# plsakr/rna-sequence-diff-patch

Measured on AMD Instinct MI355X. Metric: DP cells/sec (whole node) + edit-script bit-exact rate, 4k×4k RNA pairs, higher is better.
Workload: dtype u32

## Files before the change

### include/sed.h

```cpp
#ifndef SED_H
#define SED_H
#include <stdint.h>

#ifdef __cplusplus
extern "C" {
#endif

enum {
    SED_OK = 0,
    SED_E_ARG = -1,
    SED_E_DEVICE = -2,
    SED_E_OOM = -3,
    SED_E_RANGE = -4,
    SED_E_ALPHABET = -5,
    SED_E_STATE = -6
};

#define SED_WANT_SCRIPT 1u
#define SED_PIPELINE 2u
#define SED_NO_LEN 4u

#define SED_OPT_MODE 1
#define SED_OPT_ROWS_PER_LANE 2
#define SED_OPT_SPLIT 3
// ... 48 lines not shown
                            const uint8_t *codes_b, const int64_t *off_b, const int32_t *len_b,
                            int32_t npairs, uint32_t flags);
void sed_batch_destroy(sed_batch *b);
int sed_batch_mode(const sed_batch *b);
int sed_batch_rows_per_lane(const sed_batch *b);
int sed_batch_lane_pairs(const sed_batch *b);
int sed_batch_chains(const sed_batch *b);
int sed_batch_packed_pairs(const sed_batch *b);
int sed_batch_bitpar_pairs(const sed_batch *b);
int sed_batch_scaled_pairs(const sed_batch *b);
int sed_batch_segment_pairs(const sed_batch *b);
int sed_batch_split_tasks(const sed_batch *b);
int sed_dot_factor(const double *sub, double ins, double del, int maxmin, int ladder_maxsum, uint32_t *out);
#define SED_PLAN_ENV_TBPAR 101
#define SED_PLAN_ENV_BAND 102
#define SED_PLAN_ENV_ALT_DP 103
#define SED_PLAN_ENV_CK_HALVES 104
int sed_plan_routes(int K, const double *sub, const uint8_t *sub_int, double ins, int ins_is_int, double del,
                    int del_is_int, const int32_t *options, int noptions,
                    const uint8_t *codes_a, const int64_t *off_a, const int32_t *len_a,
                    const uint8_t *codes_b, const int64_t *off_b, const int32_t *len_b,
                    int32_t npairs, uint32_t flags, double *out, int nout);
int sed_batch_dot_keys(const sed_batch *b);
int sed_band_refine_row(int32_t n, int32_t m, int32_t rows_per_lane, double ins, double del, int32_t stripe,
                        double ub_prev, double suf, const int32_t *drow, int32_t clo_prev, int32_t chi_prev,
                        int32_t *out);
double sed_batch_band_chunks_run(sed_batch *b, double *total);
int sed_band_bounds(int32_t n, int32_t m, double ins, double del, double ub, int32_t *out);
int sed_band_chunk_range(int32_t n, int32_t m, int32_t rows_per_lane, int32_t elo, int32_t ehi, int32_t stripe,
                         int32_t *out);
double sed_band_cells(const double *sub, double ins, double del, const uint8_t *codes_a, int32_t n,
                      const uint8_t *codes_b, int32_t m, int32_t rows_per_lane);
double sed_batch_band_cells(const sed_batch *b);
int sed_batch_set_cutoff(sed_batch *b, double max_dist);
int sed_batch_cutoff_hits(sed_batch *b, int32_t *within);
int sed_batch_traceback_mode(const sed_batch *b);
int sed_batch_chain_stats(sed_batch *b, int32_t *fetched, int32_t *max_per_wave);
int sed_batch_run(sed_batch *b);
int sed_batch_sync(sed_batch *b);
int sed_batch_dp_launches(const sed_batch *b);
int sed_batch_last_times(const sed_batch *b, float *dp_ms, float *traceback_ms);
int sed_batch_times(sed_batch *b, float *dp_ms, float *traceback_ms, int max_runs);
int sed_batch_spans(sed_batch *b, float *out, int max_runs);
int sed_batch_reset_times(sed_batch *b);
int sed_batch_set_timing(sed_batch *b, int every);
int sed_batch_results(sed_batch *b, double *out_dist, uint8_t *out_is_int, int32_t *out_len,
                      uint32_t *out_ops, const int64_t *ops_off);
int sed_batch_device_results(const sed_batch *b, uint64_t *d_dist, uint64_t *d_is_int,
                             uint64_t *d_len, uint64_t *d_ops, uint64_t *ops_words);
int sed_batch_export(sed_batch *b, uint64_t d_dist, uint64_t d_len, uint64_t d_ops);
int sed_batch_work(const sed_batch *b, double *cells, double *algo_bytes);

int sed_fit_search(sed_ctx *ctx,
                   const uint8_t *codes_p, const int64_t *off_p, const int32_t *len_p,
                   const uint8_t *codes_t, const int64_t *off_t, const int32_t *len_t,
                   int32_t npairs, double *out_dist, int32_t *out_start, int32_t *out_end);
int sed_fit_plan(int K, const double *sub, const uint8_t *sub_int, double ins, int ins_is_int,
                 double del, int del_is_int, const int32_t *options, int noptions,
                 const int32_t *len_p, const int32_t *len_t, int32_t npairs, double *out, int nout);
int sed_fit_lanes(int K, const double *sub, const uint8_t *sub_int, double ins, int ins_is_int,
                  double del, int del_is_int, const int32_t *options, int noptions,
                  const int32_t *len_p, const int32_t *len_t, int32_t npairs,
                  int32_t *out_lanes, int64_t max_lanes, uint32_t *out_params);
int sed_fit_last_time(const sed_ctx *ctx, float *kernel_ms);

typedef struct sed_fit_index sed_fit_index;
// ... 34 lines not shown
```

### rna-sequence-diff-patch_amd/csrc/sed_internal.h

```cpp
#pragma once
#include <hip/hip_runtime.h>
#include <stdint.h>

#define SED_MAX_K 32

struct sed_pair_desc {
    uint64_t a_off;
    uint64_t b_off;
    uint64_t tb_off;
    uint64_t bnd_off;
    uint64_t ops_off;
    int32_t n, m;
    int32_t lane;
    int32_t map_off;
    int32_t pad[2];
};

struct sed_result {
    double dist;
    int32_t len;
    uint8_t is_int;
    uint8_t err;
    uint16_t seq;
};
// ... 53 lines not shown
    double ins, del;
    int32_t ins_int, del_int;
    int32_t K;
    uint32_t epoch;
};

struct sed_full_out {
    double *D;
    uint8_t *M;
    int32_t n, m;
};

#define SED_LAUNCH(kernel, grid, block, shmem, L, ...) \
    hipExtLaunchKernelGGL(kernel, grid, block, shmem, (L).stream, (L).ev0, (L).ev1, 0, __VA_ARGS__)

struct sed_launch {
    const sed_pair_desc *pd;
    int npairs;
    const void *seqa, *seqb;
    uint32_t *tb;
    uint32_t *ops;
    uint32_t *bnd;
    sed_result *res;
    int R;
    hipStream_t stream;
    bool tb_ladder;
    bool tb_wide;
    bool ck;
    struct sed_band *band;
    const struct sed_band_params *bandp;
    int2 *bwin;
    uint32_t *bsuf;
    int bstripes;
    hipEvent_t ev0, ev1;
    const int2 *tasks;
    int ntasks;
    const int32_t *chain_pairs, *chain_off;
    int nchains;
    uint32_t *chain_counter;
    uint32_t chain_base;
    int chain_list;
};

hipError_t sed_launch_i32(const sed_launch &L, const sed_i32_params &prm, bool len);
hipError_t sed_launch_i32_chain(const sed_launch &L, const sed_i32_params &prm, bool len);
hipError_t sed_launch_f64(const sed_launch &L, const double *gtab, const sed_f64_params &prm, bool typed);
hipError_t sed_launch_f64_seg(const sed_launch &L, const double *gtab, const sed_f64_params &prm, bool typed,
                              const int32_t *idx, int nidx);
hipError_t sed_launch_traceback_seg(const sed_launch &L, uint32_t *ops, const int32_t *idx, int nidx);
hipError_t sed_launch_f64_full(const sed_launch &L, const double *gtab, const sed_f64_params &prm, bool typed,
                               const sed_full_out &fo);
#define SED_LANE_MAXM 32
#define SED_LANE_MAXN 512
hipError_t sed_launch_lane_i32(const sed_launch &L, const int32_t *idx, int nidx, const sed_i32_params &prm, bool len);
hipError_t sed_launch_i32x2(const sed_launch &L, const int32_t *list, int nwaves, const sed_i32_params &prm);
hipError_t sed_launch_lane_i32x2(const sed_launch &L, const int32_t *idx, int nlanes, const sed_i32_params &prm);
hipError_t sed_launch_lane_bitpar(const sed_launch &L, const int32_t *idx, int nidx);
hipError_t sed_launch_lane_f64(const sed_launch &L, const int32_t *idx, int nidx, const double *gtab, double ins,
                               double del, int K, uint32_t umask);
struct sed_scaled_params {
    uint32_t row[8][2];
    uint32_t ins, del;
    double inv_scale;
    uint32_t umask, umap;
};
hipError_t sed_launch_lane_scaled(const sed_launch &L, const int32_t *idx, int nidx, const sed_scaled_params &sp);
// ... 137 lines not shown
    if (any) {
        const uint32_t us = (uint32_t)s;
        const int32_t elo = lo >= 0 ? (int32_t)(((uint32_t)lo + us - 1u) / us) : -(int32_t)((uint32_t)(-lo) / us);
        const int32_t ehi = hi >= 0 ? (int32_t)((uint32_t)hi / us) : -(int32_t)(((uint32_t)(-hi) + us - 1u) / us);
        w.elo = elo > w.elo ? elo : w.elo;
        w.ehi = ehi < w.ehi ? ehi : w.ehi;
    }
    sed_band_chunks(n, m, ROWS, nchunks, w, k, clo, chi);
    *clo = *clo > clo_prev ? *clo : clo_prev;
    *chi = *chi > chi_prev ? *chi : chi_prev;
    return any;
}
struct sed_stripe_wins {
    int2 *win;
    const uint32_t *suf;
    int stride;
};
__host__ __device__ inline double sed_band_pair_cells(int n, int m, int R, sed_band w) {
    const int ROWS = 64 * R, nstripes = sed_stripe_geom(n, m, R, 64).nstripes, nchunks = sed_stripe_geom(n, m, R, 64).nchunks;
    double cells = 0;
    for (int k = 0; k < nstripes; ++k) {
        int clo, chi;
        sed_band_chunks(n, m, ROWS, nchunks, w, k, &clo, &chi);
        const int rows = (k + 1) * ROWS < n ? ROWS : n - k * ROWS;
        const int jend = (chi >= nchunks - 1 || 64 * chi > m) ? m : 64 * chi;
        cells += (double)rows * (double)(jend - 64 * clo);
    }
    return cells;
}
struct sed_band_params {
    uint32_t cost[16];
    uint32_t ins, del;
};
hipError_t sed_launch_band(const sed_launch &L, const sed_band_params &bp);
hipError_t sed_launch_cut_band(const sed_launch &L, const int32_t *list, int nlist, uint32_t *diag,
                               const sed_band_params &bp, uint32_t tkey);
hipError_t sed_launch_i32_cut(const sed_launch &L, const int32_t *list, int nlist, const sed_i32_params &prm,
                              uint32_t tkey);
hipError_t sed_launch_cut_filter(const sed_launch &L, double cutoff, uint32_t *hits);
hipError_t sed_launch_traceback_ck(const sed_launch &L, uint32_t *ops, const sed_i32_params &prm);
hipError_t sed_launch_ck_codes(const sed_launch &L, int max_tiles, const sed_i32_params &prm);
hipError_t sed_launch_selftest(uint32_t *d_out, hipStream_t stream);
```

### rna-sequence-diff-patch_amd/csrc/sed_kernels.hip

```cpp
#include <hip/hip_ext.h>
#include <stdlib.h>
#include "sed_ck_tile.h"

template <int R> struct I32Waves { static constexpr int value = R >= 32 ? 4 : (R == 16 ? 5 : 7); };
#ifndef SED_SPLIT_BWORDS
#define SED_SPLIT_BWORDS 1024
#endif
#ifndef SED_CK_WAVES
#define SED_CK_WAVES 5
#endif
#ifndef SED_CK_GUNROLL
#define SED_CK_GUNROLL 2
#endif
#ifdef SED_I32_WAVES_PER_EU
#define SED_I32_WAVES(R) SED_I32_WAVES_PER_EU
#else
#define SED_I32_WAVES(R) I32Waves<R>::value
#endif

#define SED_SPLIT_RING 256
template <int G>
__device__ __forceinline__ void split_feed(const uint64_t *__restrict__ bin64, const int m, const int SG,
                                           const uint32_t epoch, uint32_t *ring, uint32_t *flag,
                                           const int lane) {
// ... 1280 lines not shown
    const int n = d.n, m = d.m;
    if (d.lane || n == 0 || m == 0) {
        if (lane == 0) band[pair] = sed_band{SED_BAND_OPEN_LO, SED_BAND_OPEN_HI};
        return;
    }
    const uint32_t gap = m > n ? (uint32_t)(m - n) * bp.ins : (uint32_t)(n - m) * bp.del;
    uint32_t sum = 0;
    if (suf) {
        const int len = min(n, m), words = (len + 15) >> 4, wps = ROWS >> 4;
        const uint32_t *pa = seqa + d.a_off, *pb = seqb + d.b_off;
        uint32_t *out = suf + (size_t)pair * stride;
        for (int k = (n + ROWS - 1) / ROWS - 1; k >= 0; --k) {
            uint32_t part = 0;
            for (int w = k * wps + lane; w < min(words, (k + 1) * wps); w += 64) {
                uint32_t x = pa[w], y = pb[w];
                const int cnt = min(16, len - 16 * w);
                for (int u = 0; u < cnt; ++u) {
                    part += tab[((x & 3u) << 2) | (y & 3u)];
                    x >>= 2;
                    y >>= 2;
                }
            }
#pragma unroll
            for (int o = 32; o > 0; o >>= 1) part += __shfl_xor(part, o);
            sum += part;
            if (lane == 0) out[k] = k * ROWS <= len ? sum + gap : SED_REFINE_NO_SUF;
        }
    } else {
        sum = diag_cost_sum(tab, seqa + d.a_off, seqb + d.b_off, min(n, m), lane);
    }
    if (lane == 0) band[pair] = sed_band_window(n, m, bp.ins, bp.del, (uint64_t)sum + gap);
}

__global__ __launch_bounds__(256) void sed_cut_band_kernel(const sed_pair_desc *__restrict__ pd,
                                                           const int32_t *__restrict__ list, int nlist,
                                                           const uint32_t *__restrict__ seqa,
                                                           const uint32_t *__restrict__ seqb, sed_band *__restrict__ band,
                                                           uint32_t *__restrict__ diag, sed_band_params bp, uint32_t tkey) {
    __shared__ uint32_t tab[16];
    diag_cost_table(tab, bp);
    const int lane = threadIdx.x & 63;
    const int w = blockIdx.x * 4 + (threadIdx.x >> 6);
    if (w >= nlist) return;
    const int pair = list[w];
    const sed_pair_desc d = pd[pair];
    const int n = d.n, m = d.m;
    if (n == 0 || m == 0) {
        if (lane == 0) {
            band[pair] = sed_band{SED_BAND_OPEN_LO, SED_BAND_OPEN_HI};
            if (diag) diag[pair] = 0xFFFFFFFFu;
        }
        return;
    }
    const uint32_t sum = diag_cost_sum(tab, seqa + d.a_off, seqb + d.b_off, min(n, m), lane);
    if (lane == 0) {
        const uint64_t gap = m > n ? (uint64_t)(m - n) * bp.ins : (uint64_t)(n - m) * bp.del;
        const uint64_t ub = (uint64_t)sum + gap;
        if (diag) diag[pair] = (uint32_t)(ub < 0xFFFFFFFFull ? ub : 0xFFFFFFFFull);
        band[pair] = gap > (uint64_t)tkey ? sed_band{1, 0}
                                          : sed_band_window(n, m, bp.ins, bp.del, ub < (uint64_t)tkey ? ub : (uint64_t)tkey);
    }
}

__global__ __launch_bounds__(256) void sed_cut_filter_kernel(sed_result *__restrict__ res, int npairs, double cutoff,
                                                             uint32_t *__restrict__ hits) {
    const int p = blockIdx.x * 256 + threadIdx.x;
// ... 18 lines not shown
    if (nlist <= 0) return hipSuccess;
    hipExtLaunchKernelGGL(sed_cut_band_kernel, dim3((nlist + 3) / 4), dim3(256), 0, L.stream, L.ev0, nullptr, 0, L.pd, list,
                          nlist, (const uint32_t *)L.seqa, (const uint32_t *)L.seqb, L.band, diag, bp, tkey);
    return hipGetLastError();
}
hipError_t sed_launch_i32_cut(const sed_launch &L, const int32_t *list, int nlist, const sed_i32_params &prm,
                              uint32_t tkey) {
    if (nlist <= 0 || !L.band || !L.bandp) return hipErrorInvalidValue;
    const hipError_t e = sed_launch_cut_band(L, list, nlist, nullptr, *L.bandp, tkey);
    if (e != hipSuccess) return e;
    sed_launch Lf = L;
    Lf.ev0 = nullptr;
    const dim3 grid((nlist + 3) / 4), block(256);
    const int2 *lp = reinterpret_cast<const int2 *>(list);
    const uint32_t *a = (const uint32_t *)L.seqa, *b = (const uint32_t *)L.seqb;
    switch (L.R) {
#define CASE(RR)                                                                                                        \
    case RR:                                                                                                            \
        SED_LAUNCH((sed_wf_i32_kernel<RR, false, false, false, false, false, true>), grid, block, 0, Lf, L.pd, nlist, lp, a, \
                   b, (uint32_t *)nullptr, L.bnd, L.res, prm, (const sed_band *)L.band, sed_stripe_wins{});             \
        break;
        CASE(4) CASE(8) CASE(16)
#undef CASE
    default: return hipErrorInvalidValue;
    }
    return hipGetLastError();
}
hipError_t sed_launch_cut_filter(const sed_launch &L, double cutoff, uint32_t *hits) {
    if (L.npairs <= 0) return hipSuccess;
    SED_LAUNCH(sed_cut_filter_kernel, dim3((L.npairs + 255) / 256), dim3(256), 0, L, L.res, L.npairs, cutoff, hits);
    return hipGetLastError();
}
hipError_t sed_launch_band(const sed_launch &L, const sed_band_params &bp) {
    hipExtLaunchKernelGGL(sed_band_kernel, dim3((L.npairs + 3) / 4), dim3(256), 0, L.stream, L.ev0, nullptr, 0, L.pd,
                          L.npairs, (const uint32_t *)L.seqa, (const uint32_t *)L.seqb, L.band, bp, L.bsuf, L.bstripes,
                          64 * L.R);
    return hipGetLastError();
}
template <int R, bool TB, bool LEN = true, bool CK = false, bool DOT = false>
static hipError_t launch_i32_R(const sed_launch &L, const sed_i32_params &prm) {
    if (L.ntasks > 0) {
        if constexpr (CK && R != 4) {
            return hipErrorInvalidValue;
        } else {
            SED_LAUNCH((sed_wf_i32_kernel<R, TB, true, LEN, CK, DOT>), dim3(L.ntasks), dim3(128), 0, L, L.pd, L.npairs,
                       L.tasks, (const uint32_t *)L.seqa, (const uint32_t *)L.seqb, L.tb, L.bnd, L.res, prm,
                       (const sed_band *)nullptr, sed_stripe_wins{});
        }
    } else {
        const int grid = (L.npairs + 3) / 4;
        static const int occ_lds = [] { const char *e = getenv("SED_OCC_LDS"); return e ? atoi(e) : 0; }();
        sed_launch Lf = L;
        if (CK && L.band && L.bandp) {
            const hipError_t e = sed_launch_band(L, *L.bandp);
            if (e != hipSuccess) return e;
            Lf.ev0 = nullptr;
        }
        SED_LAUNCH((sed_wf_i32_kernel<R, TB, false, LEN, CK, DOT>), dim3(grid), dim3(256), occ_lds, Lf, L.pd, L.npairs,
                           L.tasks, (const uint32_t *)L.seqa, (const uint32_t *)L.seqb, L.tb, L.bnd, L.res,
                           prm, CK ? (const sed_band *)L.band : nullptr,
                           CK && L.band ? sed_stripe_wins{L.bwin, L.bsuf, L.bstripes} : sed_stripe_wins{});
    }
    return hipGetLastError();
}

template <int R, bool TB, bool LEN, bool CK = false, int LDOT = 0>
// ... 146 lines not shown
```

### rna-sequence-diff-patch_amd/csrc/sed_plan.cpp

```cpp
#include "sed_plan.h"

#include <algorithm>
#include <climits>
#include <cmath>
#include <cstdarg>
#include <cstdio>
#include <cstring>

int sed_plan_fail(std::string *err, int code, const char *fmt, ...) {
    char buf[512];
    va_list ap;
    va_start(ap, fmt);
    vsnprintf(buf, sizeof buf, fmt, ap);
    va_end(ap);
    if (err) *err = buf;
    return code;
}

namespace {

bool is_integral_small(double v, int lim) { return v == std::floor(v) && v >= 0 && v < lim; }

struct DotKeys {
    bool ok = false;
// ... 983 lines not shown
    for (const OptSpec &s : env_table)
        if (env_keys && s.key == key) {
            o.*s.field = value;
            return true;
        }
    return false;
}

bool sed_simple_typing(const sed_costs &c) {
    if (c.ins_int || c.del_int || !(c.ins > 0) || !(c.del > 0)) return false;
    for (int e = 0; e < c.K * c.K; ++e) {
        if (c.sub_int[e] ? c.sub[e] != 0 : !(c.sub[e] > 0)) return false;
    }
    return true;
}

sed_band_params sed_band_params_from(const sed_costs &c) {
    sed_band_params bp{};
    for (int a = 0; a < 4; ++a)
        for (int bb = 0; bb < 4; ++bb)
            bp.cost[a * 4 + bb] = (a < c.K && bb < c.K) ? (uint32_t)c.sub[a * c.K + bb] : 0u;
    bp.ins = (uint32_t)c.ins;
    bp.del = (uint32_t)c.del;
    return bp;
}

uint64_t sed_band_diag_bound(const sed_band_params &bp, const uint8_t *a, int n, const uint8_t *b, int m) {
    uint64_t ub = 0;
    const int len = std::min(n, m);
    for (int i = 0; i < len; ++i) ub += bp.cost[(a[i] & 3) * 4 + (b[i] & 3)];
    return ub + (m > n ? (uint64_t)(m - n) * bp.ins : (uint64_t)(n - m) * bp.del);
}

int sed_plan_batch(const sed_costs &c, const sed_opts &o, const uint8_t *codes_a, const int64_t *off_a,
                   const int32_t *len_a, const uint8_t *codes_b, const int64_t *off_b, const int32_t *len_b,
                   int32_t npairs, uint32_t flags, sed_plan *plan, std::string *err) {
    Planning P{c, o, codes_a, off_a, len_a, codes_b, off_b, len_b, npairs, flags, *plan, err};
    int rc = plan_validate(P);
    if (rc != SED_OK) return rc;
    plan->npairs = npairs;
    plan->flags = flags;
    P.want_tb = (flags & SED_WANT_SCRIPT) != 0;
    if ((rc = plan_mode(P)) != SED_OK) return rc;
    plan_traceback(P);
    plan_layout(P);
    const bool x2_ok = plan->mode == SED_MODE_I32 && x2_costs_ok(c);
    plan_lane_routes(P, x2_ok);
    plan_wave_x2(P, x2_ok);
    plan_chain(P);
    plan_band(P);
    plan_params(P);
    plan_buffers(P);
    return SED_OK;
}

void sed_pack_sequences(const sed_plan &plan, const uint8_t *codes_a, const int64_t *off_a, const int32_t *len_a,
                        const uint8_t *codes_b, const int64_t *off_b, const int32_t *len_b, std::vector<uint32_t> &ha,
                        std::vector<uint32_t> &hb) {
    ha.assign((plan.up_copy[SED_UP_SEQA] + 3) / 4, 0);
    hb.assign((plan.up_copy[SED_UP_SEQB] + 3) / 4, 0);
    for (int p = 0; p < plan.npairs; ++p) {
        const sed_pair_desc &d = plan.pd[p];
        if (plan.mode == SED_MODE_I32) {
            pack2(codes_a + off_a[p], len_a[p], ha.data() + d.a_off);
            pack2(codes_b + off_b[p], len_b[p], hb.data() + d.b_off);
        } else {
// ... 100 lines not shown
    const int R = rows_per_lane;
    if (!out || n < 1 || m < 1 || (R != 4 && R != 8 && R != 16) || stripe < 0 || stripe >= sed_stripe_geom(n, m, R, 64).nstripes)
        return SED_E_ARG;
    const int nchunks = sed_stripe_geom(n, m, R, 64).nchunks;
    int clo, chi;
    sed_band_chunks(n, m, 64 * R, nchunks, sed_band{elo, ehi}, stripe, &clo, &chi);
    out[0] = clo;
    out[1] = chi;
    out[2] = nchunks;
    return SED_OK;
}

double sed_band_cells(const double *sub, double ins, double del, const uint8_t *codes_a, int32_t n,
                      const uint8_t *codes_b, int32_t m, int32_t rows_per_lane) {
    const int R = rows_per_lane;
    if (!sub || !codes_a || !codes_b || n < 1 || m < 1 || (R != 4 && R != 8 && R != 16) || !(ins >= 0) || !(del >= 0) ||
        !(ins + del > 0) || ins >= 65536 || del >= 65536)
        return -1.0;
    for (int i = 0; i < 16; ++i)
        if (!(sub[i] >= 0) || sub[i] >= 65536) return -1.0;
    sed_costs c;
    c.K = 4;
    c.sub.assign(sub, sub + 16);
    c.ins = ins;
    c.del = del;
    const sed_band_params bp = sed_band_params_from(c);
    for (int i = 0; i < n; ++i)
        if (codes_a[i] > 3) return -1.0;
    for (int i = 0; i < m; ++i)
        if (codes_b[i] > 3) return -1.0;
    return sed_band_pair_cells(n, m, R, sed_band_window(n, m, bp.ins, bp.del, sed_band_diag_bound(bp, codes_a, n, codes_b, m)));
}

}
```

### rna-sequence-diff-patch_amd/csrc/sed_plan.h

```cpp
#pragma once
#include "../../include/sed.h"
#include "sed_internal.h"

#include <string>
#include <vector>

struct sed_costs {
    int K = 0;
    std::vector<double> sub;
    std::vector<uint8_t> sub_int;
    double ins = 1, del = 1;
    int ins_int = 0, del_int = 0;
};

struct sed_opts {
    int mode = 0, R = 0, split = 0, lane = 0, chain = 0, pack = 0, tb = 0;
    int chain_waves = 0;
    int bitpar = 0;
    int scaled = 0;
    int seg = 0;
    int splitck = 0;
    int zc = 0;
    int dot = 0;
    int debug_corrupt = 0;
    int band = 0;
    int cut = 0;
    int fit_chunk = 0;
    int env_tbpar = -1;
    int env_band = 1;
    int env_alt_dp = 1;
    int env_ck_halves = -1;
};
bool sed_opts_set(sed_opts &o, int key, int value, bool env_keys);

int sed_plan_fail(std::string *err, int code, const char *fmt, ...);

#define SED_SMALL_BATCH_BYTES (4u << 20)

enum { SED_UP_PD, SED_UP_SEQA, SED_UP_SEQB, SED_UP_TASKS, SED_UP_CHAIN, SED_UP_LANE, SED_UP_X2, SED_UP_SEG, SED_UP_COUNT };

struct sed_plan {
    int npairs = 0;
    uint32_t flags = 0;
    int mode = 0, R = 0;
    bool split = false;
    bool ck = false;
    bool split_ck = false;
    int ck_tiles = 0;
    bool tbpar = false;
    int tbpar_items = 0, tbpar_kmax = 0;
    bool band = false;
    bool band_refine = false;
    int band_stripes = 0;
    sed_band_params bandp{};
    double band_cells = 0;
    bool cut_costs_ok = false;
    sed_band_params cut_bp{};
    bool dot = false;
    bool lad = false;
    int nlane = 0, nwave = 0;
    int nlane_x2 = 0;
    bool lane_bitpar = false;
// ... 3 lines not shown
    sed_scaled_params sp{};
    int nwave_x2 = 0;
    int nseg = 0;
    int nchains = 0;
    bool chain_dyn = false;
    size_t chain_npairs = 0;
    int ntasks = 0;
    int nbuf = 1;
    int nparts = 1;
    bool alt_dp = false;
    bool small = false, zc = false;
    uint64_t tb_words = 0, bnd_words = 0, ops_words = 0, map_words = 0;
    double cells = 0, algo_bytes = 0;
    std::vector<sed_pair_desc> pd;
    std::vector<int2> tasks;
    std::vector<int32_t> lane, seg, x2, chain;
    std::vector<int32_t> tmp;
    size_t up_size[SED_UP_COUNT] = {}, up_copy[SED_UP_COUNT] = {}, up_off[SED_UP_COUNT] = {};
    size_t res_size = 0, o_res = 0, o_ops = 0, blob_bytes = 0;
    sed_i32_params ip{};
    sed_f64_params fp{};
};

int sed_plan_batch(const sed_costs &c, const sed_opts &o, const uint8_t *codes_a, const int64_t *off_a,
                   const int32_t *len_a, const uint8_t *codes_b, const int64_t *off_b, const int32_t *len_b,
                   int32_t npairs, uint32_t flags, sed_plan *plan, std::string *err);
void sed_pack_sequences(const sed_plan &plan, const uint8_t *codes_a, const int64_t *off_a, const int32_t *len_a,
                        const uint8_t *codes_b, const int64_t *off_b, const int32_t *len_b, std::vector<uint32_t> &ha,
                        std::vector<uint32_t> &hb);

bool sed_simple_typing(const sed_costs &c);
sed_band_params sed_band_params_from(const sed_costs &c);
uint64_t sed_band_diag_bound(const sed_band_params &bp, const uint8_t *a, int n, const uint8_t *b, int m);

inline int sed_plan_chains(const sed_plan &p, bool cut_win) { return cut_win ? 0 : p.nchains; }
inline int sed_plan_traceback_mode(const sed_plan &p) {
    if (!(p.flags & SED_WANT_SCRIPT)) return 0;
    return p.ck ? 2 : p.split_ck ? 4 : (p.tbpar ? 3 : 1);
}
inline int sed_plan_dot_keys(const sed_plan &p) {
    return (p.dot ? 1 : 0) | (p.lad ? 2 : 0) | (p.lad && p.ip.lad == 2 ? 4 : 0);
}
inline int sed_plan_bitpar_pairs(const sed_plan &p) { return p.lane_bitpar ? p.nlane : p.nbitpar_f64; }
inline int sed_plan_split_tasks(const sed_plan &p) { return p.split ? p.ntasks : 0; }
inline int sed_plan_scaled_pairs(const sed_plan &p) { return p.scaled ? p.nlane - p.nbitpar_f64 : 0; }
inline int sed_plan_packed_pairs(const sed_plan &p, bool cut_win) {
    return (p.nlane_x2 > 0 ? p.nlane : 0) + (cut_win ? 0 : 2 * p.nwave_x2);
}
```

### rna-sequence-diff-patch_amd/csrc/sed_runtime.cpp

```cpp
#include "../../include/sed.h"
#include "sed_internal.h"
#include "sed_plan.h"
#include "sed_runtime.h"

#include <hip/hip_runtime.h>
#include <algorithm>
#include <array>
#include <cmath>
#include <cstdarg>
#include <cstdio>
#include <cstdlib>
#include <cstring>
#include <string>
#include <vector>

const sed_opts &sed_env_opts() {
    static const sed_opts env = [] {
        sed_opts o;
        auto knob = [](const char *name, int unset) { const char *e = getenv(name); return e ? atoi(e) : unset; };
        o.env_tbpar = knob("SED_TBPAR", -1);
        o.env_band = knob("SED_BAND", 1);
        if (const char *e = getenv("SED_BAND"))
            if (!strcmp(e, "static")) o.env_band = 3;
        o.env_alt_dp = knob("SED_ALT_DP", 1);
// ... 337 lines not shown
        ++b->runs;
        return SED_OK;
    }
    const int k = (int)(b->runs % b->plan.nbuf);
    const bool want_tb = (b->plan.flags & SED_WANT_SCRIPT) != 0;
    hipError_t e;
    if (b->plan.zc) b->zc_busy = true;
    const bool need_ev = b->plan.nbuf > 1 && !(b->plan.alt_dp && b->plan.nbuf == 2 && !want_tb);
    const bool timed = need_ev || b->time_every == 1 || (b->time_every > 1 && b->runs % b->time_every == 0);
    std::array<hipEvent_t, 4> lg{};
    if (timed) {
        if (b->nlog == b->log.size() && (e = grow_log(b, 64)) != hipSuccess) return c->hipfail(e, "event create");
        b->last_log = (long)b->nlog;
        lg = b->log[b->nlog++];
    }
    hipStream_t ts = b->plan.nbuf > 1 ? b->tb_stream : c->stream;
    const hipStream_t ds = b->plan.alt_dp && (b->runs & 1) ? b->dp2_stream : c->stream;
    sed_launch L{};
    L.pd = (const sed_pair_desc *)b->p_pd;
    L.npairs = b->plan.npairs;
    L.seqa = b->p_seqa;
    L.seqb = b->p_seqb;
    L.tb = want_tb ? (uint32_t *)b->d_tb[k].p : nullptr;
    L.ops = (uint32_t *)b->p_ops;
    L.bnd = (uint32_t *)b->d_bnd.p;
    L.res = (sed_result *)b->p_res[k];
    L.R = b->plan.R;
    L.stream = ds;
    L.tb_ladder = b->plan.mode == SED_MODE_I32 && !b->plan.split_ck;
    L.tb_wide = b->plan.lad && b->plan.ip.lad == 2;
    L.ck = b->plan.ck;
    L.band = b->plan.band ? (sed_band *)b->d_band.p : nullptr;
    L.bandp = &b->plan.bandp;
    if (L.band && b->plan.band_stripes > 0) {
        const size_t per = (size_t)b->plan.npairs * b->plan.band_stripes;
        L.bstripes = b->plan.band_stripes;
        L.bsuf = b->plan.band_refine ? (uint32_t *)b->d_bwin.p : nullptr;
        L.bwin = (int2 *)((uint32_t *)b->d_bwin.p + per);
    }
    L.tasks = b->plan.split ? (const int2 *)b->p_tasks : nullptr;
    L.ntasks = b->plan.split ? b->plan.ntasks : 0;
    const int kev = want_tb ? 3 : 1;
    if (b->plan.nbuf > 1 && (want_tb || (b->plan.alt_dp && b->plan.nbuf != 2)) && b->runs >= b->plan.nbuf &&
        hipEventQuery(b->evk[k][kev]) != hipSuccess &&
        (e = hipStreamWaitEvent(ds, b->evk[k][kev], 0)) != hipSuccess)
        return c->hipfail(e, "stream wait");
    const int nw64 = b->plan.nwave - b->plan.nseg;
    const bool cut = b->cut_on && !want_tb, win = cut && b->cut_win;
    const int ndp = (win ? 1 : (b->plan.nwave_x2 > 0) + (nw64 > 0) + (b->plan.nseg > 0)) + (b->plan.nlane > 0) + (cut ? 1 : 0);
    uint32_t *const hits = cut ? (uint32_t *)b->d_cut.p + b->cut_list.size() + (size_t)b->plan.npairs + k : nullptr;
    if (cut && (e = hipMemsetAsync(hits, 0, 4, ds)) != hipSuccess) return c->hipfail(e, "reset cutoff hits");
    b->cut_last = cut;
    int idp = 0;
    auto dp_events = [&]() {
        L.ev0 = idp == 0 ? lg[0] : nullptr;
        L.ev1 = idp == ndp - 1 ? lg[1] : nullptr;
        ++idp;
    };
    if (ndp == 0 && lg[0] && (e = hipEventRecord(lg[0], ds)) != hipSuccess) return c->hipfail(e, "event record");
    sed_i32_params ip = b->plan.ip;
    if ((e = next_split_epoch(b, ds, &ip.epoch)) != hipSuccess) return c->hipfail(e, "memset hand-off words");
    const bool len = want_tb || !(b->plan.flags & SED_NO_LEN);
    if (b->plan.nparts > 1 && want_tb) return run_batch_parts(b, lg, L, ip, len);
    if (win) {
        dp_events();
        sed_launch Lw = L;
// ... 174 lines not shown
        case SED_ERR_TB_BAND:
            return c->fail(SED_E_DEVICE, "pair %d: traceback failed: the walk left the band the forward computed", p);
        case SED_ERR_FWD_BAND:
            return c->fail(SED_E_DEVICE, "pair %d: forward failed: no cell of a stripe's boundary row fits the bound", p);
        default: return c->fail(SED_E_DEVICE, "pair %d: device error code %d", p, (int)hr[p].err);
        }
    }
    for (int p = 0; p < np; ++p) {
        if (out_dist) out_dist[p] = hr[p].dist;
        if (out_is_int) out_is_int[p] = hr[p].is_int;
        if (out_len) out_len[p] = hr[p].len;
    }
    if (want_ops)
        for (int p = 0; p < np; ++p) {
            const uint64_t words = (uint64_t)(b->plan.pd[p].n + b->plan.pd[p].m + 15) / 16;
            memcpy(out_ops + ops_off[p], hops + b->plan.pd[p].ops_off, 4 * words);
        }
    return SED_OK;
}

}

extern "C" {

const char *sed_version(void) { return "libsed 0.1 (gfx950)"; }

sed_ctx *sed_create(int device) {
    if (hipSetDevice(device) != hipSuccess) {
        (void)hipGetLastError();
        return nullptr;
    }
    sed_ctx *c = new sed_ctx();
    c->device = device;
    if (hipStreamCreateWithFlags(&c->stream, hipStreamNonBlocking) != hipSuccess) {
        (void)hipGetLastError();
        delete c;
        return nullptr;
    }
    return c;
}

void sed_destroy(sed_ctx *c) {
    if (!c) return;
    (void)hipSetDevice(c->device);
    delete c->scratch;
    c->pin.release();
    c->gtab.release();
    c->selftest.release();
    sed_fit_state_destroy(c->fit);
    if (c->stream) (void)hipStreamDestroy(c->stream);
    delete c;
}

const char *sed_last_error(const sed_ctx *c) { return c ? c->err.c_str() : "null context"; }

int sed_set_option(sed_ctx *c, int key, int value) {
    if (!c) return SED_E_ARG;
    return sed_opts_set(c->opt, key, value, false) ? SED_OK : c->fail(SED_E_ARG, "bad option %d=%d", key, value);
}

int sed_set_costs(sed_ctx *c, int K, const double *sub, const uint8_t *sub_int, double ins, int ins_is_int,
                  double del, int del_is_int) {
    if (!c) return SED_E_ARG;
    if (c->pair_pending) return c->fail(SED_E_STATE, "a submitted pair has not been waited for");
    if (K < 1 || K > 255 || !sub || !sub_int) return c->fail(SED_E_ARG, "bad cost table (K=%d)", K);
    if (!std::isfinite(ins) || !std::isfinite(del)) return c->fail(SED_E_ARG, "non-finite insert/delete cost");
// ... 519 lines not shown
```

### rna-sequence-diff-patch_amd/sedgpu.py

```python
import ctypes as C
import os
import pickle
import socket
import subprocess
import sys
import threading

import numpy as np

HERE = os.path.dirname(os.path.abspath(__file__))
LIB_PATH = os.environ.get("SED_LIBRARY", os.path.join(HERE, "libsed.so"))

SED_WANT_SCRIPT = 1
SED_PIPELINE = 2
SED_NO_LEN = 4
SED_OPT_MODE = 1
SED_OPT_ROWS_PER_LANE = 2
SED_OPT_SPLIT = 3
SED_OPT_LANE = 4
SED_OPT_CHAIN = 5
SED_OPT_PACK = 6
SED_OPT_TB = 7
SED_OPT_CHAIN_WAVES = 8
SED_OPT_DEBUG_CORRUPT = 9
# ... 14 lines not shown
SED_E_ARG = -1
SED_E_RANGE = -4

_u8p = np.ctypeslib.ndpointer(dtype=np.uint8, flags="C_CONTIGUOUS")
_i32p = np.ctypeslib.ndpointer(dtype=np.int32, flags="C_CONTIGUOUS")
_i64p = np.ctypeslib.ndpointer(dtype=np.int64, flags="C_CONTIGUOUS")
_u32p = np.ctypeslib.ndpointer(dtype=np.uint32, flags="C_CONTIGUOUS")
_f64p = np.ctypeslib.ndpointer(dtype=np.float64, flags="C_CONTIGUOUS")
_f32p = np.ctypeslib.ndpointer(dtype=np.float32, flags="C_CONTIGUOUS")

SIGNATURES = [
    ("sed_version", C.c_char_p, []),
    ("sed_create", C.c_void_p, [C.c_int]),
    ("sed_destroy", None, [C.c_void_p]),
    ("sed_last_error", C.c_char_p, [C.c_void_p]),
    ("sed_set_option", C.c_int, [C.c_void_p, C.c_int, C.c_int]),
    ("sed_set_costs", C.c_int, [C.c_void_p, C.c_int, _f64p, _u8p, C.c_double, C.c_int, C.c_double, C.c_int]),
    ("sed_run_batch", C.c_int, [C.c_void_p, _u8p, _i64p, _i32p, _u8p, _i64p, _i32p, C.c_int32, C.c_uint32,
                                _f64p, _u8p, _i32p, C.c_void_p, C.c_void_p]),
    ("sed_batch_create", C.c_void_p, [C.c_void_p, _u8p, _i64p, _i32p, _u8p, _i64p, _i32p, C.c_int32, C.c_uint32]),
    ("sed_batch_destroy", None, [C.c_void_p]),
    ("sed_batch_mode", C.c_int, [C.c_void_p]),
    ("sed_batch_rows_per_lane", C.c_int, [C.c_void_p]),
    ("sed_batch_lane_pairs", C.c_int, [C.c_void_p]),
    ("sed_batch_chains", C.c_int, [C.c_void_p]),
    ("sed_batch_dot_keys", C.c_int, [C.c_void_p]),
    ("sed_plan_routes", C.c_int, [C.c_int, _f64p, _u8p, C.c_double, C.c_int, C.c_double, C.c_int, _i32p, C.c_int,
                                  _u8p, _i64p, _i32p, _u8p, _i64p, _i32p, C.c_int32, C.c_uint32, _f64p, C.c_int]),
    ("sed_dot_factor", C.c_int, [_f64p, C.c_double, C.c_double, C.c_int, C.c_int, _u32p]),
    ("sed_band_bounds", C.c_int, [C.c_int32, C.c_int32, C.c_double, C.c_double, C.c_double, _i32p]),
    ("sed_band_chunk_range", C.c_int, [C.c_int32] * 6 + [_i32p]),
    ("sed_band_cells", C.c_double, [_f64p, C.c_double, C.c_double, _u8p, C.c_int32, _u8p, C.c_int32, C.c_int32]),
    ("sed_batch_band_cells", C.c_double, [C.c_void_p]),
    ("sed_batch_band_chunks_run", C.c_double, [C.c_void_p, _f64p]),
    ("sed_band_refine_row", C.c_int, [C.c_int32, C.c_int32, C.c_int32, C.c_double, C.c_double, C.c_int32, C.c_double,
                                      C.c_double, _i32p, C.c_int32, C.c_int32, _i32p]),
    ("sed_batch_set_cutoff", C.c_int, [C.c_void_p, C.c_double]),
    ("sed_batch_cutoff_hits", C.c_int, [C.c_void_p, C.POINTER(C.c_int32)]),
    ("sed_batch_packed_pairs", C.c_int, [C.c_void_p]),
    ("sed_batch_bitpar_pairs", C.c_int, [C.c_void_p]),
    ("sed_batch_scaled_pairs", C.c_int, [C.c_void_p]),
    ("sed_batch_segment_pairs", C.c_int, [C.c_void_p]),
    ("sed_batch_split_tasks", C.c_int, [C.c_void_p]),
    ("sed_batch_traceback_mode", C.c_int, [C.c_void_p]),
    ("sed_batch_chain_stats", C.c_int, [C.c_void_p, C.POINTER(C.c_int32), C.POINTER(C.c_int32)]),
    ("sed_batch_run", C.c_int, [C.c_void_p]),
    ("sed_batch_sync", C.c_int, [C.c_void_p]),
    ("sed_batch_last_times", C.c_int, [C.c_void_p, C.POINTER(C.c_float), C.POINTER(C.c_float)]),
    ("sed_batch_times", C.c_int, [C.c_void_p, _f32p, _f32p, C.c_int]),
    ("sed_batch_spans", C.c_int, [C.c_void_p, _f32p, C.c_int]),
    ("sed_batch_reset_times", C.c_int, [C.c_void_p]),
    ("sed_batch_set_timing", C.c_int, [C.c_void_p, C.c_int]),
    ("sed_run_pair", C.c_int, [C.c_void_p, C.c_char_p, C.c_int32, C.c_char_p, C.c_int32, C.c_uint32, C.c_void_p,
                               C.c_void_p, C.c_void_p, C.c_void_p]),
    ("sed_pair_submit", C.c_int, [C.c_void_p, C.c_char_p, C.c_int32, C.c_char_p, C.c_int32, C.c_uint32]),
    ("sed_pair_wait", C.c_int, [C.c_void_p, C.c_void_p, C.c_void_p, C.c_void_p, C.c_void_p]),
    ("sed_batch_results", C.c_int, [C.c_void_p, _f64p, _u8p, _i32p, C.c_void_p, C.c_void_p]),
    ("sed_batch_dp_launches", C.c_int, [C.c_void_p]),
    ("sed_batch_device_results", C.c_int, [C.c_void_p] + [C.POINTER(C.c_uint64)] * 5),
    ("sed_batch_export", C.c_int, [C.c_void_p, C.c_uint64, C.c_uint64, C.c_uint64]),
    ("sed_batch_work", C.c_int, [C.c_void_p, C.POINTER(C.c_double), C.POINTER(C.c_double)]),
    ("sed_fit_search", C.c_int, [C.c_void_p, _u8p, _i64p, _i32p, _u8p, _i64p, _i32p, C.c_int32, _f64p, _i32p, _i32p]),
    ("sed_fit_plan", C.c_int, [C.c_int, _f64p, _u8p, C.c_double, C.c_int, C.c_double, C.c_int, _i32p, C.c_int,
                               _i32p, _i32p, C.c_int32, _f64p, C.c_int]),
    ("sed_fit_lanes", C.c_int, [C.c_int, _f64p, _u8p, C.c_double, C.c_int, C.c_double, C.c_int, _i32p, C.c_int,
                                _i32p, _i32p, C.c_int32, _i32p, C.c_int64, _u32p]),
# ... 985 lines not shown
        err = SedError("sed_fit_index_lanes failed (%d)" % rc)
        err.code = rc
        raise err
    lanes = {k: rec[:nl, i].astype(np.int64) for i, k in enumerate(FIT_LANE_FIELDS)}
    lanes["tw"] &= 0xFFFFFFFF
    return lanes, {"row": par[:16].reshape(8, 2).copy(), "ins": int(par[16]), "del": int(par[17])}


def band_bounds(n, m, ins, dele, ub):
    out = np.zeros(2, np.int32)
    if load().sed_band_bounds(int(n), int(m), float(ins), float(dele), float(ub), out) != 0:
        raise SedError("sed_band_bounds: bad arguments")
    return int(out[0]), int(out[1])


def band_chunk_range(n, m, rows_per_lane, e_lo, e_hi, stripe):
    out = np.zeros(3, np.int32)
    if load().sed_band_chunk_range(int(n), int(m), int(rows_per_lane), int(e_lo), int(e_hi), int(stripe), out) != 0:
        raise SedError("sed_band_chunk_range: bad arguments")
    return int(out[0]), int(out[1]), int(out[2])


def band_refine_row(n, m, rows_per_lane, ins, dele, stripe, ub_prev, suf, drow, clo_prev, chi_prev):
    out = np.zeros(4, np.int32)
    row = np.ascontiguousarray(drow, np.int32)
    if len(row) != m + 1:
        raise SedError("band_refine_row: drow must hold m + 1 values")
    if load().sed_band_refine_row(int(n), int(m), int(rows_per_lane), float(ins), float(dele), int(stripe), float(ub_prev),
                                  -1.0 if suf is None else float(suf), row, int(clo_prev), int(chi_prev), out) != 0:
        raise SedError("sed_band_refine_row: bad arguments")
    return int(out[0]), int(out[1]), int(out[2]), bool(out[3])


def band_cells(sub, ins, dele, codes_a, codes_b, rows_per_lane=16):
    a, b = np.ascontiguousarray(codes_a, np.uint8), np.ascontiguousarray(codes_b, np.uint8)
    r = load().sed_band_cells(np.ascontiguousarray(sub, np.float64).ravel(), float(ins), float(dele), a, len(a), b, len(b),
                              int(rows_per_lane))
    if r < 0:
        raise SedError("sed_band_cells: bad arguments")
    return float(r)
```

Measured before the change: 29360 billion.

## Tighten band upper bound with per-segment narrow-band DP kernel

```diff
diff --git a/include/sed.h b/include/sed.h
--- a/include/sed.h
+++ b/include/sed.h
@@ -104,6 +104,8 @@
 double sed_band_cells(const double *sub, double ins, double del, const uint8_t *codes_a, int32_t n,
                       const uint8_t *codes_b, int32_t m, int32_t rows_per_lane);
 double sed_batch_band_cells(const sed_batch *b);
+double sed_band_seg_ub(const double *sub, double ins, double del, const uint8_t *codes_a, int32_t n,
+                       const uint8_t *codes_b, int32_t m, int32_t seg_rows, int32_t half_width, double *suf, int32_t nsuf);
 int sed_batch_set_cutoff(sed_batch *b, double max_dist);
 int sed_batch_cutoff_hits(sed_batch *b, int32_t *within);
 int sed_batch_traceback_mode(const sed_batch *b);
diff --git a/rna-sequence-diff-patch_amd/csrc/sed_internal.h b/rna-sequence-diff-patch_amd/csrc/sed_internal.h
--- a/rna-sequence-diff-patch_amd/csrc/sed_internal.h
+++ b/rna-sequence-diff-patch_amd/csrc/sed_internal.h
@@ -109,6 +109,7 @@
     int2 *bwin;
     uint32_t *bsuf;
     int bstripes;
+    bool bseg;
     hipEvent_t ev0, ev1;
     const int2 *tasks;
     int ntasks;
@@ -312,6 +313,8 @@
     uint32_t cost[16];
     uint32_t ins, del;
 };
+#define SED_BAND_SEG_H 256
+#define SED_BAND_SEG_W 8
 hipError_t sed_launch_band(const sed_launch &L, const sed_band_params &bp);
 hipError_t sed_launch_cut_band(const sed_launch &L, const int32_t *list, int nlist, uint32_t *diag,
                                const sed_band_params &bp, uint32_t tkey);
diff --git a/rna-sequence-diff-patch_amd/csrc/sed_kernels.hip b/rna-sequence-diff-patch_amd/csrc/sed_kernels.hip
--- a/rna-sequence-diff-patch_amd/csrc/sed_kernels.hip
+++ b/rna-sequence-diff-patch_amd/csrc/sed_kernels.hip
@@ -1336,6 +1336,87 @@
     if (lane == 0) band[pair] = sed_band_window(n, m, bp.ins, bp.del, (uint64_t)sum + gap);
 }
 
+#ifndef SED_BAND_SEG_PRIO
+#define SED_BAND_SEG_PRIO 2
+#endif
+__global__ __launch_bounds__(256) void sed_band_seg_kernel(const sed_pair_desc *__restrict__ pd, int npairs,
+                                                           const uint32_t *__restrict__ seqa,
+                                                           const uint32_t *__restrict__ seqb, sed_band *__restrict__ band,
+                                                           sed_band_params bp, uint32_t *__restrict__ suf, int stride,
+                                                           int ROWS, int lshift) {
+    constexpr int W = SED_BAND_SEG_W, H = SED_BAND_SEG_H, NB = 2 * W + 1;
+    constexpr uint32_t BIG = 0x3FFFFFFFu;
+    static_assert(W == 8 && H % 16 == 0, "the 64-bit symbol window holds 16 rows of 2 W + 1 = 17 symbols");
+    __shared__ uint32_t tab[16];
+    __shared__ uint32_t segc[256];
+    if constexpr (SED_BAND_SEG_PRIO > 0) __builtin_amdgcn_s_setprio(SED_BAND_SEG_PRIO);
+    diag_cost_table(tab, bp);
+    const int t = threadIdx.x, s = t & ((1 << lshift) - 1);
+    const int pair = blockIdx.x * (256 >> lshift) + (t >> lshift);
+    int n = 0, m = 0;
+    bool stripe_pair = false;
+    uint32_t a_off = 0, b_off = 0;
+    if (pair < npairs) {
+        const sed_pair_desc d = pd[pair];
+        n = d.n, m = d.m, a_off = d.a_off, b_off = d.b_off;
+        stripe_pair = !(d.lane || n == 0 || m == 0);
+    }
+    const int len = min(n, m), rs = s * H;
+    const int rows = stripe_pair && rs < len ? min(H, len - rs) : 0;
+    uint32_t cost = 0;
+    if (rows > 0) {
+        const uint32_t *pa = seqa + a_off, *pb = seqb + b_off;
+        const int bwords = (m + 15) >> 4;
+        const uint32_t indel = bp.ins + bp.del;
+        uint32_t u[NB];
+#pragma unroll
+        for (int x = 0; x < NB; ++x) u[x] = x < W ? BIG : 0u;
+        int x0 = rs >> 4;
+        uint32_t prev = x0 > 0 ? pb[x0 - 1] : 0u, cur = pb[x0], aw = 0;
+        uint64_t win = 0;
+        for (int rr = 0; rr < rows; ++rr) {
+            if ((rr & 15) == 0) {
+                const uint32_t next = x0 + 1 < bwords ? pb[x0 + 1] : 0u;
+                aw = pa[x0];
+                win = (uint64_t)(prev >> 16) | ((uint64_t)cur << 16) | ((uint64_t)(next & 0xFFFFu) << 48);
+                prev = cur;
+                cur = next;
+                ++x0;
+            }
+            const uint32_t a4 = (aw & 3u) << 2;
+            uint32_t c[NB];
+#pragma unroll
+            for (int x = 0; x < NB; ++x) c[x] = tab[a4 | ((uint32_t)(win >> (2 * x)) & 3u)];
+            uint32_t left = BIG;
+#pragma unroll
+            for (int x = 0; x < NB; ++x) {
+                uint32_t v = min(u[x] + c[x], left);
+                if (x + 1 < NB) v = min(v, u[x + 1] + indel);
+                u[x] = left = v;
+            }
+            aw >>= 2;
+            win >>= 2;
+        }
+        cost = u[W];
+    }
+    segc[t] = cost;
+    __syncthreads();
+    if (s != 0 || pair >= npairs) return;
+    if (!stripe_pair) {
+        band[pair] = sed_band{SED_BAND_OPEN_LO, SED_BAND_OPEN_HI};
+        return;
+    }
+    const uint32_t gap = m > n ? (uint32_t)(m - n) * bp.ins : (uint32_t)(n - m) * bp.del;
+    const int sps = ROWS / H;
+    const uint32_t *mine = segc + (t & ~((1 << lshift) - 1));
+    uint32_t sum = 0;
+    for (int k = (n + ROWS - 1) / ROWS - 1; k >= 0; --k) {
+        for (int q = 0; q < sps; ++q) sum += mine[k * sps + q];
+        if (suf) suf[(size_t)pair * stride + k] = k * ROWS <= len ? sum + gap : SED_REFINE_NO_SUF;
+    }
+    band[pair] = sed_band_window(n, m, bp.ins, bp.del, (uint64_t)sum + gap);
+}
+
 __global__ __launch_bounds__(256) void sed_cut_band_kernel(const sed_pair_desc *__restrict__ pd,
                                                            const int32_t *__restrict__ list, int nlist,
                                                            const uint32_t *__restrict__ seqa,
@@ -1420,6 +1501,16 @@
     return hipGetLastError();
 }
 hipError_t sed_launch_band(const sed_launch &L, const sed_band_params &bp) {
+    const int ROWS = 64 * L.R, segs = (L.bstripes > 0 ? L.bstripes : 1) * (ROWS / SED_BAND_SEG_H);
+    if (L.bseg && ROWS % SED_BAND_SEG_H == 0 && segs <= 256) {
+        int lshift = 0;
+        while ((1 << lshift) < segs) ++lshift;
+        const int ppb = 256 >> lshift;
+        hipExtLaunchKernelGGL(sed_band_seg_kernel, dim3((L.npairs + ppb - 1) / ppb), dim3(256), 0, L.stream, L.ev0, nullptr,
+                              0, L.pd, L.npairs, (const uint32_t *)L.seqa, (const uint32_t *)L.seqb, L.band, bp, L.bsuf,
+                              L.bstripes, ROWS, lshift);
+        return hipGetLastError();
+    }
     hipExtLaunchKernelGGL(sed_band_kernel, dim3((L.npairs + 3) / 4), dim3(256), 0, L.stream, L.ev0, nullptr, 0, L.pd,
                           L.npairs, (const uint32_t *)L.seqa, (const uint32_t *)L.seqb, L.band, bp, L.bsuf, L.bstripes,
                           64 * L.R);
diff --git a/rna-sequence-diff-patch_amd/csrc/sed_plan.cpp b/rna-sequence-diff-patch_amd/csrc/sed_plan.cpp
--- a/rna-sequence-diff-patch_amd/csrc/sed_plan.cpp
+++ b/rna-sequence-diff-patch_amd/csrc/sed_plan.cpp
@@ -1039,6 +1039,38 @@
     return ub + (m > n ? (uint64_t)(m - n) * bp.ins : (uint64_t)(n - m) * bp.del);
 }
 
+uint64_t sed_band_seg_bound(const sed_band_params &bp, const uint8_t *a, int n, const uint8_t *b, int m, int H, int w,
+                            uint64_t *suf) {
+    const int len = std::min(n, m), nseg = (len + H - 1) / H;
+    const uint64_t INF = ~0ull >> 2, gap = m > n ? (uint64_t)(m - n) * bp.ins : (uint64_t)(n - m) * bp.del;
+    std::vector<uint64_t> seg(nseg), row(2 * w + 1), nxt(2 * w + 1);
+    for (int s = 0; s < nseg; ++s) {
+        const int rs = s * H, re = std::min(len, rs + H);
+        for (int e = -w; e <= w; ++e) row[e + w] = e >= 0 && rs + e <= re ? (uint64_t)e * bp.ins : INF;
+        for (int i = rs + 1; i <= re; ++i) {
+            for (int e = -w; e <= w; ++e) {
+                const int j = i + e;
+                uint64_t v = INF;
+                if (j >= rs && j <= re) {
+                    if (j > rs && row[e + w] < INF) v = row[e + w] + bp.cost[(a[i - 1] & 3) * 4 + (b[j - 1] & 3)];
+                    if (e < w && row[e + 1 + w] < INF) v = std::min(v, row[e + 1 + w] + bp.del);
+                    if (e > -w && j > rs && nxt[e - 1 + w] < INF) v = std::min(v, nxt[e - 1 + w] + bp.ins);
+                }
+                nxt[e + w] = v;
+            }
+            row.swap(nxt);
+        }
+        seg[s] = row[w];
+    }
+    uint64_t sum = gap;
+    if (suf) suf[nseg] = sum;
+    for (int s = nseg - 1; s >= 0; --s) {
+        sum += seg[s];
+        if (suf) suf[s] = sum;
+    }
+    return sum;
+}
+
 int sed_plan_batch(const sed_costs &c, const sed_opts &o, const uint8_t *codes_a, const int64_t *off_a,
                    const int32_t *len_a, const uint8_t *codes_b, const int64_t *off_b, const int32_t *len_b,
                    int32_t npairs, uint32_t flags, sed_plan *plan, std::string *err) {
@@ -1205,4 +1237,28 @@
     return sed_band_pair_cells(n, m, R, sed_band_window(n, m, bp.ins, bp.del, sed_band_diag_bound(bp, codes_a, n, codes_b, m)));
 }
 
-}
+double sed_band_seg_ub(const double *sub, double ins, double del, const uint8_t *codes_a, int32_t n,
+                       const uint8_t *codes_b, int32_t m, int32_t seg_rows, int32_t half_width, double *suf, int32_t nsuf) {
+    if (!sub || !codes_a || !codes_b || n < 1 || m < 1 || seg_rows < 1 || half_width < 0 || half_width > 4096 ||
+        !(ins >= 0) || !(del >= 0) || !(ins + del > 0) || ins >= 65536 || del >= 65536)
+        return -1.0;
+    const int nseg = (std::min(n, m) + seg_rows - 1) / seg_rows;
+    if (suf ? nsuf != nseg + 1 : nsuf != 0) return -1.0;
+    for (int i = 0; i < 16; ++i)
+        if (!(sub[i] >= 0) || sub[i] >= 65536) return -1.0;
+    for (int i = 0; i < n; ++i)
+        if (codes_a[i] > 3) return -1.0;
+    for (int i = 0; i < m; ++i)
+        if (codes_b[i] > 3) return -1.0;
+    sed_costs c;
+    c.K = 4;
+    c.sub.assign(sub, sub + 16);
+    c.ins = ins;
+    c.del = del;
+    std::vector<uint64_t> s64(nseg + 1);
+    const uint64_t ub = sed_band_seg_bound(sed_band_params_from(c), codes_a, n, codes_b, m, seg_rows, half_width, s64.data());
+    for (int s = 0; suf && s <= nseg; ++s) suf[s] = (double)s64[s];
+    return (double)ub;
+}
+
+}
diff --git a/rna-sequence-diff-patch_amd/csrc/sed_plan.h b/rna-sequence-diff-patch_amd/csrc/sed_plan.h
--- a/rna-sequence-diff-patch_amd/csrc/sed_plan.h
+++ b/rna-sequence-diff-patch_amd/csrc/sed_plan.h
@@ -28,6 +28,7 @@
     int fit_chunk = 0;
     int env_tbpar = -1;
     int env_band = 1;
+    int env_band_ub = 1;
     int env_alt_dp = 1;
     int env_ck_halves = -1;
 };
@@ -97,6 +98,8 @@
 bool sed_simple_typing(const sed_costs &c);
 sed_band_params sed_band_params_from(const sed_costs &c);
 uint64_t sed_band_diag_bound(const sed_band_params &bp, const uint8_t *a, int n, const uint8_t *b, int m);
+uint64_t sed_band_seg_bound(const sed_band_params &bp, const uint8_t *a, int n, const uint8_t *b, int m, int H, int w,
+                            uint64_t *suf);
 
 inline int sed_plan_chains(const sed_plan &p, bool cut_win) { return cut_win ? 0 : p.nchains; }
 inline int sed_plan_traceback_mode(const sed_plan &p) {
diff --git a/rna-sequence-diff-patch_amd/csrc/sed_runtime.cpp b/rna-sequence-diff-patch_amd/csrc/sed_runtime.cpp
--- a/rna-sequence-diff-patch_amd/csrc/sed_runtime.cpp
+++ b/rna-sequence-diff-patch_amd/csrc/sed_runtime.cpp
@@ -393,6 +393,7 @@
     L.ck = b->plan.ck;
     L.band = b->plan.band ? (sed_band *)b->d_band.p : nullptr;
     L.bandp = &b->plan.bandp;
+    L.bseg = c->opt.env_band_ub != 0;
     if (L.band && b->plan.band_stripes > 0) {
         const size_t per = (size_t)b->plan.npairs * b->plan.band_stripes;
         L.bstripes = b->plan.band_stripes;
@@ -633,6 +634,7 @@
     }
     sed_ctx *c = new sed_ctx();
     c->device = device;
+    if (const char *e = getenv("SED_BAND_UB")) c->opt.env_band_ub = strcmp(e, "diag") ? 1 : 0;
     if (hipStreamCreateWithFlags(&c->stream, hipStreamNonBlocking) != hipSuccess) {
         (void)hipGetLastError();
         delete c;
diff --git a/rna-sequence-diff-patch_amd/sedgpu.py b/rna-sequence-diff-patch_amd/sedgpu.py
--- a/rna-sequence-diff-patch_amd/sedgpu.py
+++ b/rna-sequence-diff-patch_amd/sedgpu.py
@@ -70,6 +70,8 @@
     ("sed_band_chunk_range", C.c_int, [C.c_int32] * 6 + [_i32p]),
     ("sed_band_cells", C.c_double, [_f64p, C.c_double, C.c_double, _u8p, C.c_int32, _u8p, C.c_int32, C.c_int32]),
     ("sed_batch_band_cells", C.c_double, [C.c_void_p]),
+    ("sed_band_seg_ub", C.c_double, [_f64p, C.c_double, C.c_double, _u8p, C.c_int32, _u8p, C.c_int32, C.c_int32, C.c_int32,
+                                     _f64p, C.c_int32]),
     ("sed_batch_band_chunks_run", C.c_double, [C.c_void_p, _f64p]),
     ("sed_band_refine_row", C.c_int, [C.c_int32, C.c_int32, C.c_int32, C.c_double, C.c_double, C.c_int32, C.c_double,
                                       C.c_double, _i32p, C.c_int32, C.c_int32, _i32p]),
@@ -1121,6 +1123,16 @@
     return int(out[0]), int(out[1]), int(out[2]), bool(out[3])
 
 
+def band_seg_bound(sub, ins, dele, codes_a, codes_b, seg_rows=256, half_width=8):
+    a, b = np.ascontiguousarray(codes_a, np.uint8), np.ascontiguousarray(codes_b, np.uint8)
+    suf = np.zeros((min(len(a), len(b)) + int(seg_rows) - 1) // max(int(seg_rows), 1) + 1, np.float64)
+    r = load().sed_band_seg_ub(np.ascontiguousarray(sub, np.float64).ravel(), float(ins), float(dele), a, len(a), b, len(b),
+                               int(seg_rows), int(half_width), suf, len(suf))
+    if r < 0:
+        raise SedError("sed_band_seg_ub: bad arguments")
+    return float(r), suf
+
+
 def band_cells(sub, ins, dele, codes_a, codes_b, rows_per_lane=16):
     a, b = np.ascontiguousarray(codes_a, np.uint8), np.ascontiguousarray(codes_b, np.uint8)
     r = load().sed_band_cells(np.ascontiguousarray(sub, np.float64).ravel(), float(ins), float(dele), a, len(a), b, len(b),
```

Result: no change. 29330 billion (median of 3 runs) (-0.1%).
